# denyingmxd/CFPNet

Measured on AMD Instinct MI355X. Metric: depth maps/sec @ 480x640 bf16 (whole job; per_gpu = value / n_gpus); abs_rel vs CPU oracle, higher is better.
Workload: dtype bf16; 1 GPU; batch=8 480x640 RGB + 8x8-zone ToF, eval forward incl. the prob output [B,256,H/2,W/2] written in the storage dtype (bf16: 2 bytes/element); layers=hist2image combine1 image x2 (CFPNet), parallelism=single GPU

## Files before the change

cfpnet_amd/engine.py:

```python
from __future__ import annotations

import math
import os
from typing import Dict, List, Optional, Sequence, Tuple

import torch

from . import hip, ops, spec
from .geometry import FUSION_SCALES, FusionGeometry, gsa_keys, static_zone_key, zone_records as _zone_records
from .ops import Act

_BN_EPS = 1e-5


def _same_pad(size: int, k: int, s: int) -> Tuple[int, int]:
    total = max((math.ceil(size / s) - 1) * s + k - size, 0)
    return total // 2, total - total // 2


_STREAMS: Dict = {}
_CONCURRENT: Dict[str, list] = {}


def concurrent_streams(device, want: int = 4, pool: int = 16) -> list:
# ... 291 lines not shown
            bufs[key] = (torch.zeros if zero else torch.empty)(shape, dtype=dtype, device=self.device)
        assert tuple(bufs[key].shape) == tuple(shape), key
        return bufs[key]

    def _f32(self, plan, key: str, n: int) -> torch.Tensor:
        bufs = plan["bufs"]
        if key not in bufs:
            bufs[key] = torch.empty(max(n, 1), dtype=torch.float32, device=self.device)
        assert bufs[key].numel() >= n, key
        return bufs[key]

    def _cv(self, name, x: Act, out: Act, B, H, W, k, stride=1, pads=None, act=hip.ACT_NONE, residual=None):
        if pads is None:
            p = (k - 1) // 2
            pt = pl = p
            Ho, Wo = (H + 2 * p - k) // stride + 1, (W + 2 * p - k) // stride + 1
        else:
            (pt, pb), (pl, pr) = pads
            Ho, Wo = (H + pt + pb - k) // stride + 1, (W + pl + pr - k) // stride + 1
        ops.conv2d(x, self.P[name + ".w"], self.P[name + ".s"], self.P[name + ".t"], out, B, H, W, k, k, stride, pt, pl,
                   Ho, Wo, act, residual, self._ws(B * Ho * Wo, out.C, k * k * x.C))
        return Ho, Wo

    def _lin(self, wname, x: Act, out: Act, rows, act=hip.ACT_NONE, residual=None, st: Optional[str] = None, ln=None):
        ops.linear(x, self.P[wname], self.P[st + ".s"] if st else None, self.P[st + ".t"] if st else None, out, rows, act, residual,
                   None if ln is not None else self._ws(rows, out.C, x.C), ln)

    def _ws(self, M: int, Cout: int, K: int) -> Optional[torch.Tensor]:
        need = ops.conv2d_ws_bytes(M, Cout, K, self.cdt)
        if need == 0:
            return None
        if self.tickets:
            need += hip.CONV_TICKET_BYTES
        ws = self._lane_ws.get(self._lane)
        if ws is None or ws.numel() * 4 < need:
            if self._capturing:
                raise RuntimeError("split-K workspace must be sized by a warm-up forward before graph capture")
            if self.tickets:
                ws = ops.ticket_ws(need - hip.CONV_TICKET_BYTES, self.device)
            else:
                ws = torch.empty((need + 3) // 4, dtype=torch.float32, device=self.device)
            self._lane_ws[self._lane] = ws
        return ws

    def _dbg(self, name: str, a: Act):
        if self._dbg_round:
            for pat, dt in self._dbg_round.items():
                if name == pat or (pat.endswith("*") and name.startswith(pat[:-1])):
                    t = a.torch()
                    t.copy_(t.to(dt).to(t.dtype))

    def _encoder(self, plan, rgb: torch.Tensor, B, H, W, taps):
        e = "img_encoder"
        x8 = self._act(plan, "rgb8", B * H * W, 8)
        (ops.rgb_to_nhwc8_hilo if self.rgb_hilo else ops.rgb_to_nhwc8)(rgb, x8, B, H, W)
        pads = (_same_pad(H, 3, 2), _same_pad(W, 3, 2))
        h, w = math.ceil(H / 2), math.ceil(W / 2)
        x = self._act(plan, "stem", B * h * w, spec.ENC_STEM_OUT)
        self._cv("stem", x8, x, B, H, W, 3, 2, pads, hip.ACT_SILU if self.stem_act else hip.ACT_NONE)
        self._dbg("stem", x)
        tap_acts: List[Act] = []
        for bi, b in enumerate(spec.ENC_BLOCKS):
            q = f"{e}.{b.prefix}"
            ho, wo = math.ceil(h / b.stride), math.ceil(w / b.stride)
            pads = (_same_pad(h, 3, b.stride), _same_pad(w, 3, b.stride))
            if bi in spec.ENC_TAPS:
                out = plan["tap_dst"][spec.ENC_TAPS[bi]]
            else:
                out = self._act(plan, f"enc{bi}", B * ho * wo, b.cout)
            res = x if b.skip else None
            if b.kind == "cn":
                self._cv(q + ".conv", x, out, B, h, w, 3, b.stride, pads, hip.ACT_SILU, res)
            elif b.kind == "er":
                if (self.half and (q + ".pwl.wp") in self.P and ("1" if b.stride == 1 else "2") in self.er_fused and taps is None
                        and not self._dbg_round and ops.conv3x3_pw_fused_variant(x.C, b.mid, b.cout, b.stride, ops.DT[self.dtype]) >= 0):
                    ops.conv3x3_pw_fused(x, self.P[q + ".exp.w"], self.P[q + ".exp.s"], self.P[q + ".exp.t"], hip.ACT_SILU, self.P[q + ".pwl.wp"],
                                         self.P[q + ".pwl.s"], self.P[q + ".pwl.t"], out, B, h, w, b.stride, pads[0][0], pads[1][0], ho, wo,
                                         hip.ACT_NONE, res)
                else:
                    mid = self._act(plan, f"enc{bi}.mid", B * ho * wo, b.mid)
                    self._cv(q + ".exp", x, mid, B, h, w, 3, b.stride, pads, hip.ACT_SILU)
                    self._dbg(f"enc{bi}.mid", mid)
                    self._cv(q + ".pwl", mid, out, B, ho, wo, 1, 1, None, hip.ACT_NONE, res)
            else:
                mid2 = self._act(plan, f"enc{bi}.dw", B * ho * wo, b.mid)
                mbp = ops.mbconv_plan(B, h, w, x.C, b.mid) if (q + ".pw.wimg") in self.P else None
                if mbp is not None:
                    ns = mbp[0]
                    part = self._f32(plan, f"enc{bi}.sum", B * ns * b.mid)
                    ops.mbconv_expand_dw(x, self.P[q + ".pw.wimg"], self.P[q + ".pw.s"], self.P[q + ".pw.t"], self.P[q + ".dw.w"],
                                         self.P[q + ".dw.s"], self.P[q + ".dw.t"], mid2, part, B, h, w)
                elif ((self.se2 or self.se2_x3 == "1" or (self.se2_x3 == "auto" and not ops.PLAN_IN_FLIGHT)) and b.se_rd <= 64
                      and ops.dwconv3x3_se_parts(B, ho, wo, b.mid, b.stride, ops.DT[self.dtype]) > 0):
                    mid = self._act(plan, f"enc{bi}.mid", B * h * w, b.mid)
                    self._cv(q + ".pw", x, mid, B, h, w, 1, 1, None, hip.ACT_SILU)
                    K = ops.dwconv3x3_se_parts(B, ho, wo, b.mid, b.stride, ops.DT[self.dtype])
                    hpart = self._f32(plan, f"enc{bi}.hpart", B * K * b.se_rd)
                    ops.dwconv3x3_se(mid, self.P[q + ".dw.w"], self.P[q + ".dw.s"], self.P[q + ".dw.t"], mid2, self.P[q + ".se.wr"], hpart,
                                     B, h, w, b.stride, pads[0][0], pads[1][0], ho, wo, hip.ACT_SILU)
                    if self.x3:
                        wb = self._buf(plan, f"enc{bi}.wb", (B, b.cout, (b.mid + 31) // 32 * 64), torch.float16, zero=True)
                    else:
                        wb = self._buf(plan, f"enc{bi}.wb", (B, b.cout, b.mid), self.dtype)
                    ops.se_gate_fold2(hpart, K, 1.0 / (ho * wo), self.P[q + ".se.br"], self.P[q + ".se.we_t"], self.P[q + ".se.be"],
                                      self.P[q + ".pwl.w32"], wb, B, b.cout, b.mid, b.se_rd, x3=self.x3)
                    ops.conv2d(mid2, wb, self.P[q + ".pwl.s"], self.P[q + ".pwl.t"], out, B, ho, wo, 1, 1, 1, 0, 0, ho, wo, hip.ACT_NONE,
                               res, self._piw_ws(plan, bi, B, ho * wo, b.cout, b.mid), per_image_weights=True)
                    x, h, w = out, ho, wo
                    if bi in spec.ENC_TAPS:
                        tap_acts.append(out)
                        if taps is not None:
                            taps[f"enc{spec.ENC_TAPS[bi]}"] = self._nchw(out, B, h, w)
                    continue
                else:
                    mid = self._act(plan, f"enc{bi}.mid", B * h * w, b.mid)
                    self._cv(q + ".pw", x, mid, B, h, w, 1, 1, None, hip.ACT_SILU)
                    ns = ops.dwconv3x3_strips(B, ho, wo, b.mid, b.stride, ops.DT[self.dtype])
                    part = self._f32(plan, f"enc{bi}.sum", B * ns * b.mid)
                    self._dbg(f"enc{bi}.mid", mid)
                    ops.dwconv3x3_sum(mid, self.P[q + ".dw.w"], self.P[q + ".dw.s"], self.P[q + ".dw.t"], mid2, part, B, h, w, b.stride,
                                      pads[0][0], pads[1][0], ho, wo, hip.ACT_SILU)
                    self._dbg(f"enc{bi}.dw", mid2)
# ... 722 lines not shown
```

cfpnet_amd/hip.py:

```python
from __future__ import annotations

import ctypes as C
import os
from typing import Optional

_HERE = os.path.dirname(os.path.abspath(__file__))
LIB_PATH = os.environ.get("CFP_HIP_LIB") or os.path.join(_HERE, "libcfpnet_hip.so")

F32, BF16, F16 = 0, 1, 2
F32X3 = 3
ACT_NONE, ACT_RELU, ACT_LRELU, ACT_SILU, ACT_GELU, ACT_SIGMOID = range(6)
TOF_SAMPLE_UNIFORM, TOF_SAMPLE_ICDF = 0, 1
HEAD_WOUT_HILO, HEAD_RAM_HILO = 1, 2
UNC_STD, UNC_ENTROPY, UNC_PMAX = 0, 1, 2
SPARS_STD, SPARS_ENTROPY, SPARS_PMAX, SPARS_ORACLE_RMSE, SPARS_ORACLE_ABSREL = range(5)
RENDER_DEPTH, RENDER_GT, RENDER_ABS_ERR, RENDER_REL_ERR = range(4)
REGION_ALL, REGION_FOV_IN, REGION_FOV_OUT, REGION_ZONE_VALID, REGION_ZONE_INVALID = range(5)
CONV_PER_IMAGE, CONV_W2, CONV_IN_FLIGHT, CONV_X3, CONV_WS_TICKETS = 1, 2, 4, 8, 16
CONV_TICKET_BYTES = 4096

_p, _i, _f, _sz, _ll = C.c_void_p, C.c_int, C.c_float, C.c_size_t, C.c_longlong

SIGNATURES = {
    "cfp_version": (_i, []),
    "cfp_last_error": (C.c_char_p, []),
    "cfp_conv2d_nhwc": (_i, [_p, _i, _p, _p, _p, _p, _i, _p, _i] + [_i] * 14 + [_p, _sz, _p]),
    "cfp_conv2d_nhwc_ex": (_i, [_p, _i, _p, _p, _p, _p, _i, _p, _i] + [_i] * 14 + [_p, _p, _f, _i, _p, _sz, _p]),
    "cfp_conv2d_nhwc_moments": (_i, [_p, _i, _p, _p, _p, _i] + [_i] * 13 + [_p, _sz, _p, _sz, _p, _p, _p]),
    "cfp_conv2d_ws_bytes": (_sz, [_i, _i, _i, _i]),
    "cfp_pack_w_x3_elems": (_sz, [_ll, _i]),
    "cfp_pack_w_x3": (_i, [_p, _p, _ll, _i, _p]),
    "cfp_conv2d_plan": (_i, [_i] * 8 + [_p, _p]),
    "cfp_debug_set": (_i, [_i, _i]),
    "cfp_conv2d_variant": (_i, [_i, _i]),
    "cfp_dwconv3x3_nhwc": (_i, [_p, _i, _p, _p, _p, _p, _i] + [_i] * 11 + [_p]),
    "cfp_dwconv3x3_strips": (_i, [_i] * 6),
    "cfp_dwconv3x3_launch_slots": (_i, [_i] * 10),
    "cfp_dwconv3x3_sum_nhwc": (_i, [_p, _i, _p, _p, _p, _p, _i, _p] + [_i] * 11 + [_p]),
    "cfp_se_fold": (_i, [_p, _p, _p, _p, _p, _i, _i, _i, _i, _i, _p]),
    "cfp_se_gate_fold": (_i, [_p, _i, _f, _p, _p, _p, _p, _p, _p, _i, _i, _i, _i, _i, _p]),
    "cfp_dwconv3x3_se_parts": (_i, [_i, _i, _i, _i, _i, _i]),
    "cfp_dwconv3x3_se_nhwc": (_i, [_p, _i, _p, _p, _p, _p, _i, _p, _i, _p] + [_i] * 11 + [_p]),
    "cfp_se_gate_fold2": (_i, [_p, _i, _f, _p, _p, _p, _p, _p, _i, _i, _i, _i, _i, _p]),
    "cfp_dwconv_large_nhwc": (_i, [_p, _i, _p, _p, _p, _p, _i] + [_i] * 7 + [_p]),
    "cfp_dwconv_large_toeplitz_elems": (_sz, [_i, _i]),
    "cfp_dwconv_large_toeplitz": (_i, [_p, _p, _i, _i, _i, _i, _p]),
    "cfp_dwconv_large_mfma_nhwc": (_i, [_p, _i, _p, _p, _p, _p, _i] + [_i] * 7 + [_p]),
    "cfp_channel_sum": (_i, [_p, _i, _p, _i, _i, _i, _i, _i, _p]),
    "cfp_se_hidden": (_i, [_p, _i, _f, _p, _p, _p, _i, _i, _i, _p]),
    "cfp_se_scale": (_i, [_p, _i, _p, _p, _p, _i, _i, _i, _i, _i, _p]),
    "cfp_scale_channels": (_i, [_p, _i, _p, _i, _i, _i, _i, _p]),
    "cfp_layernorm": (_i, [_p, _i, _p, _p, _f, _p, _i, _p, _i, _i, _i, _i, _p]),
    "cfp_attn_kv_ws_floats": (_sz, [_i] * 7),
    "cfp_attn_kv_reduce": (_i, [_p, _i, _p, _i, _p, _p, _p] + [_i] * 10 + [_f, _i, _i, _i, _p]),
    "cfp_attn_apply": (_i, [_p, _i, _p, _p, _p, _i] + [_i] * 9 + [_f, _f, _i, _i, _i, _p]),
    "cfp_loftr_tail": (_i, [_p, _i, _p, _p, _p, _i, _p, _i, _p, _p, _p, _p, _p, _p, _p, _p, _f] + [_i] * 5 + [_f, _f, _i, _i, _i, _p]),
    "cfp_loftr_tail_x2i": (_i, [_p, _p, _p, _i, _i, _i, _i, _i] + [_p] * 8 + [_f] + [_i] * 5 + [_p, _i, _i, _f, _f, _i, _i, _i, _p]),
    "cfp_resize_bilinear": (_i, [_p, _i] + [_i] * 6 + [_p, _i] + [_i] * 6 + [_p] + [_i] * 7 + [_p]),
    "cfp_resize_bilinear_dev": (_i, [_p, _i, _i, _i, _p, _i, _i, _i, _p, _i, _p] + [_i] * 6 + [_i, _p]),
    "cfp_attn_kv_reduce_dev": (_i, [_p, _i, _p, _i, _p, _p, _p] + [_i] * 5 + [_p, _i, _i, _i, _i, _p]),
    "cfp_attn_kv_project_fits": (_i, [_i] * 8),
    "cfp_attn_kv_project_reduce": (_i, [_p, _i, _p, _p, _p, _p] + [_i] * 10 + [_f, _i, _i, _i, _p]),
    "cfp_attn_kv_project_reduce_dev": (_i, [_p, _i, _p, _p, _p, _p] + [_i] * 5 + [_p, _i, _i, _i, _i, _p]),
    "cfp_attn_apply_dev": (_i, [_p, _i, _p, _p, _p, _i] + [_i] * 5 + [_p, _f, _i, _i, _i, _p]),
    "cfp_add_rowtable": (_i, [_p, _i, _p, _p, _i] + [_i] * 8 + [_p]),
    "cfp_upsample_cat_conv3x3": (_i, [_p, _i, _i, _i, _i, _p, _i, _i, _p, _p, _p, _p, _i] + [_i] * 6 + [_p]),
# ... 45 lines not shown
    "cfp_bn_train_stats_partials": (_i, [_p, _i, C.c_longlong, C.c_longlong, _i, _p, _p, _f, _f] + [_p] * 7 + [_p]),
    "cfp_scale_shift_act": (_i, [_p, _i, _p, _p, _i, _p, _i, C.c_longlong, _i, _i, _p]),
    "cfp_scale_shift_act_res": (_i, [_p, _i, _p, _p, _i, _p, _i, _p, _i, C.c_longlong, _i, _i, _p]),
    "cfp_bn_train_bwd": (_i, [_p, _i, _p, _i, C.c_longlong, _i, _i, _p, _p, _p, _p, _i, _p, _p, _p, _i, _p, _sz, _p]),
    "cfp_colsum": (_i, [_p, _i, C.c_longlong, _i, _i, _p, _p, _sz, _p]),
    "cfp_act_bwd": (_i, [_p, _i, _p, _i, _i, _p, _i, C.c_longlong, _i, _i, _p]),
    "cfp_layernorm_bwd_ws_bytes": (_sz, [C.c_longlong, _i]),
    "cfp_layernorm_bwd": (_i, [_p, _i, _p, _i, _p, _f, _p, _i, _i, _p, _p, C.c_longlong, _i, _i, _p, _sz, _p]),
    "cfp_layernorm_bwd_deferred": (_i, [_p, _i, _p, _i, _p, _f, _p, _i, _i, _p, _p, C.c_longlong, _i, _i, _p, _sz, _p, _p]),
    "cfp_axpby": (_i, [_p, _i, _p, _i, _f, _f, _p, _i, C.c_longlong, _i, _i, _p]),
    "cfp_rowtable_grad": (_i, [_p, _i, _p, _i, _i, _i, _i, _i, _i, _i, _f, _i, _p]),
    "cfp_se_train_ws_floats": (_sz, [_i, _i, _i]),
    "cfp_se_train_fwd": (_i, [_p, _i, _f] + [_p] * 7 + [_i, _i, _i, _p]),
    "cfp_se_train_bwd": (_i, [_p] * 12 + [_f, _f, _i, _i, _i, _p]),
    "cfp_channel_dot": (_i, [_p, _i, _p, _i, _p, _i, _i, _i, _i, _p]),
    "cfp_bcast_fma": (_i, [_p, _i, _p, _p, _p, _i, _i, _i, _i, _i, _p]),
    "cfp_dwconv3x3_dgrad": (_i, [_p, _i, _p, _p, _i] + [_i] * 11 + [_p]),
    "cfp_dwconv3x3_wgrad_ws_bytes": (_sz, [_i]),
    "cfp_dwconv3x3_wgrad": (_i, [_p, _i, _p, _i, _p] + [_i] * 9 + [_f, _i, _p, _sz, _p]),
    "cfp_dwconv3x3_wgrad_deferred": (_i, [_p, _i, _p, _i, _p] + [_i] * 9 + [_f, _i, _p, _sz, _p, _p]),
    "cfp_index_rows": (_i, [_p, _i, _p, _p, _i, C.c_longlong, _i, _i, _i, _p]),
    "cfp_resize_bilinear_bwd": (_i, [_p, _i, _p, _i, _i, _i, _i, _i, _i, _i, _i, _i, _p]),
    "cfp_bin_centers": (_i, [_p, _f, _f, _p, _p, _i, _i, _p]),
    "cfp_bin_centers_bwd": (_i, [_p, _f, _f, _p, _i, _i, _p]),
    "cfp_softmax_expect_ws_bytes": (_sz, [_i, _i, _i]),
    "cfp_softmax_expect": (_i, [_p, _i, _p, _p, _p, _p, _i, _p, _i, _i, _i, _i, _p, _sz, _p]),
    "cfp_linattn_state_bytes": (_sz, [_i, _i, _i]),
    "cfp_linattn_ws_bytes": (_sz, [_i, _i, _i, _i, _i]),
    "cfp_linattn_fwd": (_i, [_p, _i, _p, _i, _p, _i, _p, _i, _p, _i, _i, _i, _i, _i, _f, _i, _p, _sz, _p]),
    "cfp_linattn_bwd": (_i, [_p, _i, _p, _i, _p, _i, _p, _i, _p, _p, _i, _p, _i, _p, _i, _i, _i, _i, _i, _i, _f, _i, _p, _sz, _p]),
    "cfp_linattn_fwd_dev": (_i, [_p, _i, _p, _i, _p, _i, _p, _i, _p, _i, _i, _i, _i, _i, _f, _i, _p, _sz, _p, _p]),
    "cfp_linattn_bwd_dev": (_i, [_p, _i, _p, _i, _p, _i, _p, _i, _p, _p, _i, _p, _i, _p, _i, _i, _i, _i, _i, _i, _f, _i, _p, _sz, _p, _p]),
    "cfp_zone_crop": (_i, [_p, _i, _p, _p, _i] + [_i] * 7 + [_i, _p]),
    "cfp_zone_crop_bwd": (_i, [_p, _i, _p, _p, _i] + [_i] * 7 + [_i, _p]),
    "cfp_zone_paste": (_i, [_p, _i, _p, _i, _p, _p, _i] + [_i] * 7 + [_i, _p]),
    "cfp_zone_paste_bwd": (_i, [_p, _i, _p, _p, _i] + [_i] * 7 + [_i, _p]),
    "cfp_zone_rect_rows": (_i, [_p, _i, _p, _p, _i] + [_i] * 6 + [_i, _p]),
    "cfp_dwconv_large_wgrad_ws_bytes": (_sz, [_i, _i, _i, _i, _i]),
    "cfp_dwconv_large_wgrad": (_i, [_p, _i, _p, _i, _p, _i, _i, _i, _i, _i, _f, _i, _p, _sz, _p]),
    "cfp_row_normalize": (_i, [_p, _p, _p, _i, _i, _p]),
    "cfp_add_rowtable_dev": (_i, [_p, _i, _p, _p, _i, _i, _i, _i, _i, _i, _i, _p, _i, _p]),
    "cfp_rowtable_grad_dev": (_i, [_p, _i, _p, _i, _i, _i, _i, _i, _i, _p, _f, _i, _p]),
    "cfp_nyu_augment": (_i, [_p, _p, _i, _i, _i, _p, _p, _p, _i, _i, C.POINTER(C.c_float), C.POINTER(C.c_float), _p, _p, _p]),
    "cfp_nyu_rotate": (_i, [_p, _p, _p, _p, _i, _i, _i, _p, _p]),
    "cfp_bin_regressor": (_i, [_p, _i, _f] + [_p] * 7 + [_f, _f, _i, _p, _p, _i, _i, _i, _i, _p]),
    "cfp_bin_softmax": (_i, [_p, _i, _p, _p, _p, _i, _i, _i, _i, _p]),
    "cfp_bin_softmax_stats": (_i, [_p, _i, _p, _p, _p, _p, _i, _i, _i, _i, _p]),
    "cfp_conv3x3_mean": (_i, [_p, _i, _p, _i, _p, _p, _p, _i, _i, _i, _i, _i, _i, _p]),
    "cfp_lkpm_tail": (_i, [_p, _i, _p, _i, _p, _i, _p, _p, _p, _p, _p, _p, _f, _i, _i, _i, _p]),
    "cfp_mbconv_plan": (_i, [_i, _i, _i, _i, _i, _p, _p]),
    "cfp_mbconv_expand_dw": (_i, [_p, _i, _p, _p, _p, _p, _p, _p, _p, _i, _p, _i, _i, _i, _i, _i, _i, _p]),
    "cfp_conv3x3_pw_fused_variant": (_i, [_i] * 5),
    "cfp_conv3x3_chunk_variant": (_i, [_i] * 4),
    "cfp_conv3x3_pw_fused": (_i, [_p, _i, _p, _p, _p, _i, _p, _p, _p, _i, _p, _i, _p, _i] + [_i] * 12 + [_p]),
    "cfp_hist_encoder": (_i, [_p, _p, _p, _p, _p, _p, _p, _p, _p, _i, _i, _i, _p]),
    "cfp_depth_head_fused": (_i, [_p, _i, _p, _p, _p, _p, _p, _p, _p, _p, _p, _i, _i, _i, _i, _i, _p]),
    "cfp_bin_head_fused": (_i, [_p, _i, _p, _p, _p, _p, _p, _i, _i, _i, _i, _p]),
    "cfp_depth_head_conv0_fused": (_i, [_p, _i, _p, _p, _p, _p, _p, _p, _p, _p, _p, _p, _p, _i, _i, _i, _i, _i, _p]),
    "cfp_depth_head_fused_stats": (_i, [_p, _i, _p, _p, _p, _p, _p, _p, _p, _p, _p, _p, _i, _i, _i, _i, _i, _p]),
    "cfp_bin_head_fused_stats": (_i, [_p, _i, _p, _p, _p, _p, _p, _p, _i, _i, _i, _i, _p]),
}

class WgradJob(C.Structure):
    _fields_ = [("slabs", C.c_void_p), ("dw", C.c_void_p), ("db", C.c_void_p), ("n", C.c_longlong), ("n_dw", C.c_longlong),
                ("nsplit", C.c_int), ("ew", C.c_int), ("beta", C.c_float), ("beta_b", C.c_float)]


_lib: Optional[C.CDLL] = None


def load() -> C.CDLL:
    global _lib
    if _lib is not None:
        return _lib
    if not os.path.exists(LIB_PATH):
        raise RuntimeError(
            f"{LIB_PATH} not found: build the HIP extension first "
            f"(`python -c 'import __graft_entry__ as g; g.build()'` or `make -C cfpnet_amd/csrc`). "
            "There is no CPU fallback for the product path.")
    import torch
    lib = C.CDLL(LIB_PATH)
    for name, (res, args) in SIGNATURES.items():
        fn = getattr(lib, name)
        fn.restype = res
        fn.argtypes = args
    _lib = lib
    return lib


def last_error() -> str:
    return load().cfp_last_error().decode()


def call(name: str, *args):
    rc = getattr(load(), name)(*args)
    if rc != 0:
        raise RuntimeError(f"{name} failed ({rc}): {last_error()}")


def ptr(t) -> int:
    return 0 if t is None else t.data_ptr()


def current_stream() -> int:
    import torch
    return torch.cuda.current_stream().cuda_stream
# ... 1 lines not shown
```

cfpnet_amd/ops.py:

```python
from __future__ import annotations

import os
from dataclasses import dataclass
from typing import Optional, Tuple

import torch

from . import hip

DT = {torch.float32: hip.F32, torch.bfloat16: hip.BF16, torch.float16: hip.F16}


@dataclass
class Act:
    buf: torch.Tensor
    c0: int
    C: int

    @property
    def rows(self) -> int:
        return self.buf.shape[0]

    @property
    def ld(self) -> int:
# ... 385 lines not shown
        hip.call("cfp_resize_bilinear_dev", src.ptr, src.ld, Hs, Ws, dst.ptr, dst.ld, Hd, Wd, _rec_ptr(rec), int(rec_side),
                 hip.ptr(zone_valid), zn, p1, p2, int(accumulate), B, src.C, src.dt, _s())
        return
    sy0, sx0, sh, sw = srect
    dy0, dx0, dh, dw = drect
    hip.call("cfp_resize_bilinear", src.ptr, src.ld, Hs, Ws, sy0, sx0, sh, sw, dst.ptr, dst.ld, Hd, Wd, dy0, dx0, dh, dw,
             hip.ptr(zone_valid), zn, p1, p2, int(accumulate), B, src.C, src.dt, _s())


def add_rowtable(x: Act, table, out: Act, rows, H, W, Wt, oy, ox):
    assert table.dtype == torch.float32 and table.shape[1] == x.C
    hip.call("cfp_add_rowtable", x.ptr, x.ld, table.data_ptr(), out.ptr, out.ld, rows, x.C, H, W, Wt, oy, ox, x.dt, _s())


def copy_rows(x: Act, out: Act, rows):
    hip.call("cfp_copy_rows", x.ptr, x.ld, out.ptr, out.ld, rows, x.C, x.dt, _s())


def upsample_cat_conv3x3(low: Act, Hs, Ws, skip: Act, w, scale, shift, out: Act, B, H, W, act, x3: bool = False):
    if x3:
        assert low.dt == skip.dt == out.dt == hip.F32 and w.dtype == torch.float16 and w.shape[-1] == 9 * (low.C + (skip.C + 31) // 32 * 32) * 2
        hip.call("cfp_upsample_cat_conv3x3", low.ptr, low.ld, Hs, Ws, low.C, skip.ptr, skip.ld, skip.C, w.data_ptr(),
                 hip.ptr(scale), hip.ptr(shift), out.ptr, out.ld, B, H, W, out.C, act, hip.F32X3, _s())
        return
    assert w.shape[-1] == 9 * (low.C + skip.C) and low.dt == skip.dt == out.dt
    hip.call("cfp_upsample_cat_conv3x3", low.ptr, low.ld, Hs, Ws, low.C, skip.ptr, skip.ld, skip.C, w.data_ptr(),
             hip.ptr(scale), hip.ptr(shift), out.ptr, out.ld, B, H, W, out.C, act, out.dt, _s())


def pack_w_x3_cat(w: torch.Tensor, cup: int) -> torch.Tensor:
    co, kh, kw, cin = w.shape
    assert kh == 3 and kw == 3 and cup % 32 == 0 and 0 < cup < cin
    csk = cin - cup
    pad = (csk + 31) // 32 * 32 - csk
    wp = torch.nn.functional.pad(w, (0, pad)) if pad else w
    return pack_w_x3(wp.reshape(co, 9 * (cup + csk + pad)).contiguous())


def copy_rows2(x0: Act, out0: Act, x1: Act, out1: Act, rows):
    assert x0.dt == x1.dt == out0.dt == out1.dt and out0.C == x0.C and out1.C == x1.C
    hip.call("cfp_copy_rows2", x0.ptr, x0.ld, out0.ptr, out0.ld, x0.C, x1.ptr, x1.ld, out1.ptr, out1.ld, x1.C, rows, x0.dt, _s())


def rgb_to_nhwc8(rgb: torch.Tensor, out: Act, B, H, W):
    assert rgb.dtype == torch.float32 and rgb.is_contiguous() and out.C == 8 and out.ld == 8
    hip.call("cfp_rgb_to_nhwc8", rgb.data_ptr(), out.ptr, B, H, W, out.dt, _s())


def rgb_to_nhwc8_hilo(rgb: torch.Tensor, out: Act, B, H, W):
    assert rgb.dtype == torch.float32 and rgb.is_contiguous() and out.C == 8 and out.ld == 8
    hip.call("cfp_rgb_to_nhwc8_hilo", rgb.data_ptr(), out.ptr, B, H, W, out.dt, _s())


def scalar_to_rows8(x: torch.Tensor, out: Act, rows):
    assert x.dtype == torch.float32 and x.is_contiguous() and out.C == 8 and out.ld == 8
    hip.call("cfp_scalar_to_rows8", x.data_ptr(), out.ptr, rows, out.dt, _s())


def bin_regressor(partial, nsplit, inv_hw, w1x1, w0, b0, w1, b1, w2, b2, min_val, max_val, norm, edges, centers, B, C,
                  hidden, nbins):
    hip.call("cfp_bin_regressor", partial.data_ptr(), nsplit, float(inv_hw), w1x1.data_ptr(), w0.data_ptr(), b0.data_ptr(),
             w1.data_ptr(), b1.data_ptr(), w2.data_ptr(), b2.data_ptr(), float(min_val), float(max_val), norm,
             edges.data_ptr(), centers.data_ptr(), B, C, hidden, nbins, _s())


def _check_stats(stats, B, HW):
    assert stats.dtype == torch.float32 and stats.is_contiguous() and stats.numel() == B * 3 * HW, "stats: float32 [B, 3, HW]"


def bin_softmax(logits: Act, centers, prob, pred, B, HW, nbins, stats=None):
    if stats is None:
        hip.call("cfp_bin_softmax", logits.ptr, logits.ld, centers.data_ptr(), hip.ptr(prob), pred.data_ptr(), B, HW, nbins,
                 logits.dt, _s())
        return
    _check_stats(stats, B, HW)
    hip.call("cfp_bin_softmax_stats", logits.ptr, logits.ld, centers.data_ptr(), hip.ptr(prob), pred.data_ptr(), stats.data_ptr(), B, HW,
             nbins, logits.dt, _s())


def bin_head_fused(x: Act, w, bias, centers, prob, pred, B, HW, stats=None):
    x3 = x.buf.dtype == torch.float32 and w.dtype == torch.float16
    assert not x3 or (tuple(w.shape) == (256, (x.C + 31) // 32 * 64) and (prob is None or prob.dtype == torch.float32))
    if stats is None:
        hip.call("cfp_bin_head_fused", x.ptr, x.ld, w.data_ptr(), bias.data_ptr(), centers.data_ptr(), hip.ptr(prob),
                 pred.data_ptr(), B, HW, x.C, hip.F32X3 if x3 else x.dt, _s())
        return
    _check_stats(stats, B, HW)
    hip.call("cfp_bin_head_fused_stats", x.ptr, x.ld, w.data_ptr(), bias.data_ptr(), centers.data_ptr(), hip.ptr(prob),
             pred.data_ptr(), stats.data_ptr(), B, HW, x.C, hip.F32X3 if x3 else x.dt, _s())


def permute_wout(w: torch.Tensor, dtype, hilo: bool = True, diffuse: bool = False) -> torch.Tensor:
    w = w.detach().float().reshape(w.shape[0], -1)
    assert w.shape == (256, 128)
    src = pw_k_order(128)
    wp = w[:, src]
    hi = (round_taps(w.reshape(256, 1, 128), dtype).reshape(256, 128)[:, src] if diffuse else wp).to(dtype)
    planes = [hi]
    if hilo:
        planes.append((wp - hi.float()).to(dtype))
    return torch.stack(planes).contiguous()


def pw_k_order(K: int) -> torch.Tensor:
    pos = torch.arange((K + 31) // 32 * 32)
    kb, q, e = pos // 32, (pos % 32) // 8, pos % 8
# ... 103 lines not shown
```

include/cfpnet_hip.h:

```cpp
#ifndef CFPNET_HIP_H
#define CFPNET_HIP_H

#include <stddef.h>
#include <stdint.h>

#ifdef __cplusplus
extern "C" {
#endif

typedef void* cfp_stream_t;

enum { CFP_OK = 0, CFP_EINVAL = -1, CFP_ESHAPE = -2, CFP_EHIP = -3 };
enum { CFP_F32 = 0, CFP_BF16 = 1, CFP_F16 = 2 };
enum { CFP_F32X3 = 3 };
enum { CFP_TOF_SAMPLE_UNIFORM = 0, CFP_TOF_SAMPLE_ICDF = 1 };
enum { CFP_ACT_NONE = 0, CFP_ACT_RELU = 1, CFP_ACT_LRELU = 2, CFP_ACT_SILU = 3, CFP_ACT_GELU = 4, CFP_ACT_SIGMOID = 5 };

int cfp_version(void);
const char* cfp_last_error(void);

int cfp_conv2d_nhwc(const void* in, int in_ld, const void* w, const float* scale, const float* shift,
                    const void* residual, int res_ld, void* out, int out_ld,
                    int B, int H, int W, int Cin, int Cout, int KH, int KW, int stride,
                    int pad_t, int pad_l, int Ho, int Wo, int act, int dtype,
// ... 14 lines not shown
size_t cfp_conv2d_ws_bytes(int M, int Cout, int K, int dtype);

int cfp_conv2d_plan(int M, int Cout, int K, int KH, int stride, int dtype, int rows_per_batch, int B, int* variant,
                    int* splits);

int cfp_conv3x3_chunk_variant(int M, int Cin, int Cout, int in_flight);

int cfp_conv2d_variant(int M, int Cout);

int cfp_debug_set(int key, int value);

int cfp_dwconv3x3_nhwc(const void* in, int in_ld, const void* w, const float* scale, const float* shift,
                       void* out, int out_ld, int B, int H, int W, int C, int stride, int pad_t, int pad_l,
                       int Ho, int Wo, int act, int dtype, cfp_stream_t stream);

int cfp_dwconv3x3_strips(int B, int Ho, int Wo, int C, int stride, int dtype);
int cfp_dwconv3x3_launch_slots(int B, int H, int W, int Ho, int Wo, int C, int stride, int in_ld, int out_ld, int dtype);
int cfp_dwconv3x3_sum_nhwc(const void* in, int in_ld, const void* w, const float* scale, const float* shift,
                           void* out, int out_ld, float* partial, int B, int H, int W, int C, int stride,
                           int pad_t, int pad_l, int Ho, int Wo, int act, int dtype, cfp_stream_t stream);

int cfp_dwconv_large_nhwc(const void* in, int in_ld, const float* w, const float* scale, const float* shift,
                          void* out, int out_ld, int B, int H, int W, int C, int k, int act, int dtype,
                          cfp_stream_t stream);

size_t cfp_dwconv_large_toeplitz_elems(int C, int k);
int cfp_dwconv_large_toeplitz(const float* w, void* out, int C, int k, int flip, int dtype, cfp_stream_t stream);
int cfp_dwconv_large_mfma_nhwc(const void* in, int in_ld, const void* toeplitz, const float* scale, const float* shift,
                               void* out, int out_ld, int B, int H, int W, int C, int k, int act, int dtype,
                               cfp_stream_t stream);

int cfp_channel_sum(const void* in, int in_ld, float* partial, int B, int HW, int C, int nsplit, int dtype,
                    cfp_stream_t stream);

int cfp_se_hidden(const float* partial, int nsplit, float inv_hw, const float* w_reduce, const float* b_reduce,
                  float* hidden, int B, int C, int R, cfp_stream_t stream);

int cfp_se_scale(void* x, int ld, const float* hidden, const float* w_expand_t, const float* b_expand,
                 int B, int HW, int C, int R, int dtype, cfp_stream_t stream);

int cfp_se_fold(const void* w_proj, void* w_out, const float* hidden, const float* w_expand_t, const float* b_expand,
                int B, int Cout, int C, int R, int dtype, cfp_stream_t stream);

int cfp_mbconv_plan(int B, int H, int W, int Cin, int mid, int* tiles_per_image, int* KP);
int cfp_mbconv_expand_dw(const void* x, int x_ld, const void* wpw, const float* s1, const float* t1, const void* wdw,
                         const float* s2, const float* t2, void* out, int out_ld, float* partial, int B, int H, int W, int Cin,
                         int mid, int dtype, cfp_stream_t stream);

int cfp_conv3x3_pw_fused_variant(int Cin, int Cmid, int Cout, int stride, int dtype);
int cfp_conv3x3_pw_fused(const void* in, int in_ld, const void* w1, const float* scale1, const float* shift1, int act1,
                         const void* w2_pad, const float* scale2, const float* shift2, int act2, const void* residual, int res_ld,
                         void* out, int out_ld, int B, int H, int W, int Cin, int Cmid, int Cout, int stride, int pad_t, int pad_l,
                         int Ho, int Wo, int dtype, cfp_stream_t stream);

int cfp_se_gate_fold(const float* partial, int nsplit, float inv_hw, const float* w_reduce, const float* b_reduce,
                     const float* w_expand_t, const float* b_expand, const void* w_proj, void* w_out,
                     int B, int Cout, int C, int R, int dtype, cfp_stream_t stream);

int cfp_dwconv3x3_se_parts(int B, int Ho, int Wo, int C, int stride, int dtype);
int cfp_dwconv3x3_se_nhwc(const void* in, int in_ld, const void* w, const float* scale, const float* shift, void* out, int out_ld,
                          const float* w_reduce, int R, float* hpart, int B, int H, int W, int C, int stride, int pad_t, int pad_l,
                          int Ho, int Wo, int act, int dtype, cfp_stream_t stream);

int cfp_se_gate_fold2(const float* hpart, int K, float inv_hw, const float* b_reduce, const float* w_expand_t, const float* b_expand,
                      const float* w_proj, void* w_out, int B, int Cout, int C, int R, int dtype, cfp_stream_t stream);

int cfp_scale_channels(void* x, int ld, const float* gate, int B, int HW, int C, int dtype, cfp_stream_t stream);

int cfp_layernorm(const void* in, int in_ld, const float* gamma, const float* beta, float eps,
                  const void* residual, int res_ld, void* out, int out_ld, int rows, int C, int dtype,
                  cfp_stream_t stream);

size_t cfp_attn_kv_ws_floats(int NB, int Hk, int Wk, int th, int tw, int heads, int d);
int cfp_attn_kv_reduce(const void* k, int k_ld, const void* v, int v_ld, float* kv, float* ksum, float* ws,
                       int NB, int Hk, int Wk, int th, int tw, int cy0, int cy1, int cx0, int cx1,
                       int count_pad, float v_length, int heads, int d, int dtype, cfp_stream_t stream);

int cfp_attn_kv_reduce_dev(const void* k, int k_ld, const void* v, int v_ld, float* kv, float* ksum, float* ws,
                           int NB, int Hk, int Wk, int th, int tw, const int* rec, int count_pad, int heads, int d, int dtype,
                           cfp_stream_t stream);

int cfp_attn_kv_project_fits(int NB, int Hk, int Wk, int th, int tw, int heads, int d, int dtype);
int cfp_attn_kv_project_reduce(const void* x, int x_ld, const void* w_kv, float* kv, float* ksum, float* ws,
                               int NB, int Hk, int Wk, int th, int tw, int cy0, int cy1, int cx0, int cx1,
                               int count_pad, float v_length, int heads, int d, int dtype, cfp_stream_t stream);
int cfp_attn_kv_project_reduce_dev(const void* x, int x_ld, const void* w_kv, float* kv, float* ksum, float* ws,
                                   int NB, int Hk, int Wk, int th, int tw, const int* rec, int count_pad, int heads, int d, int dtype,
                                   cfp_stream_t stream);

int cfp_attn_apply(const void* q, int q_ld, const float* kv, const float* ksum, void* out, int out_ld,
                   int NB, int Hq, int Wq, int qth, int qtw, int ey0, int ey1, int ex0, int ex1,
                   float v_length, float eps, int heads, int d, int dtype, cfp_stream_t stream);

int cfp_attn_apply_dev(const void* q, int q_ld, const float* kv, const float* ksum, void* out, int out_ld,
                       int NB, int Hq, int Wq, int qth, int qtw, const int* rec, float eps, int heads, int d, int dtype,
                       cfp_stream_t stream);

int cfp_loftr_tail(const void* q, int q_ld, const float* kv, const float* ksum, const void* x, int x_ld,
                   void* out, int out_ld, const void* w_q, const void* w_merge, const void* w_mlp0, const void* w_mlp2,
                   const float* ln1_g, const float* ln1_b, const float* ln2_g, const float* ln2_b, float ln_eps,
                   int NB, int Hq, int Wq, int qth, int qtw, float v_length, float eps, int heads, int D,
                   int dtype, cfp_stream_t stream);

int cfp_loftr_tail_x2i(const float* kv, const float* ksum, void* tok, int tok_ld, int H, int W, int sy, int sx,
                       const void* w_q, const void* w_merge, const void* w_mlp0, const void* w_mlp2,
                       const float* ln1_g, const float* ln1_b, const float* ln2_g, const float* ln2_b, float ln_eps,
// ... 286 lines not shown
```

Measured before the change: 4093 maps/s.

## Fuse RGB hi/lo packing, stem conv and first encoder conv into one kernel

Adds a HIP kernel that reads fp32 RGB directly, splits it into hi/lo half-precision pairs in LDS, runs the stride-2 stem 3x3 conv with MFMA into an LDS tile with halo, then runs the first 3x3 conv block from LDS and writes only its 16-channel output. This removes the rgb8 and 40-channel stem activation round trips through global memory and two kernel launches. In exchange it recomputes the stem on halo pixels per tile and uses a large LDS footprint, which may limit occupancy. It is enabled by default for half dtypes with hilo RGB, and an environment variable can turn it off.

```diff
diff --git a/cfpnet_amd/csrc/stem_fused.hip b/cfpnet_amd/csrc/stem_fused.hip
--- /dev/null
+++ b/cfpnet_amd/csrc/stem_fused.hip
@@ -0,0 +1,270 @@
+#include "halo_core.h"
+
+namespace {
+
+constexpr int kC0 = 40, kK0 = 72;
+constexpr int kC1 = 16, kK1 = 9 * kC0;
+constexpr int kPP = 96;
+constexpr int kRC = 37;
+constexpr int kW0Bytes = kC0 * kK0 * 2, kW1Bytes = kC1 * kK1 * 2;
+constexpr int kNK = 2 * kC0 + 2 * kC1;
+
+struct StemP {
+  const float* rgb;
+  const void* w0;
+  const float *s0, *t0;
+  const void* w1;
+  const float *s1, *t1;
+  void* out;
+  int out_ld, H, W, Hs, Ws, tiles_x, tiles_y, act0, act1;
+  int probe;
+};
+
+template <int TH> struct StemTile {
+  static constexpr int SR = TH + 2, SPIX = SR * 18;
+  static constexpr int RR = 2 * SR + 1, RPIX = RR * kRC;
+  static constexpr int S_BYTES = SPIX * kPP, RGB_BYTES = RPIX * 16;
+  static constexpr int K_OFF = S_BYTES + (RGB_BYTES + kW0Bytes > kW1Bytes ? RGB_BYTES + kW0Bytes : kW1Bytes);
+  static constexpr int LDS = K_OFF + kNK * 4;
+};
+
+template <typename H, int TH>
+__global__ __launch_bounds__(256) void stem_fused_kernel(StemP p) {
+  using T = StemTile<TH>;
+  constexpr int SPIX = T::SPIX, RPIX = T::RPIX;
+  constexpr int NR = (RPIX + 255) / 256;
+  constexpr int RW = TH / 4;
+  static_assert(kW1Bytes / 16 <= 3 * 256 && kW0Bytes / 16 <= 2 * 256, "weight pieces per thread");
+  __shared__ __attribute__((aligned(16))) unsigned char smem[T::LDS];
+  unsigned char* sS = smem;
+  unsigned char* sR = smem + T::S_BYTES;
+  unsigned char* sW0 = sR + T::RGB_BYTES;
+  unsigned char* sW1 = sR;
+  float* sK = reinterpret_cast<float*>(smem + T::K_OFF);
+
+  const int tid = threadIdx.x;
+  const int lane = tid & 63;
+  const int wave = __builtin_amdgcn_readfirstlane(tid >> 6);
+  const int fr = lane & 15, fq = lane >> 4;
+
+  int bid = xcd_remap(blockIdx.x, gridDim.x);
+  const int x0 = (bid % p.tiles_x) * 16; bid /= p.tiles_x;
+  const int y0 = (bid % p.tiles_y) * TH;
+  const int b = bid / p.tiles_y;
+  const int HW = p.H * p.W;
+
+  u32x4 w1r[3], w0r[2];
+#pragma unroll
+  for (int n = 0; n < 3; ++n) {
+    const int i = tid + n * 256;
+    w1r[n] = i < kW1Bytes / 16 ? reinterpret_cast<const u32x4*>(p.w1)[i] : u32x4{0u, 0u, 0u, 0u};
+  }
+#pragma unroll
+  for (int n = 0; n < 2; ++n) {
+    const int i = tid + n * 256;
+    w0r[n] = i < kW0Bytes / 16 ? reinterpret_cast<const u32x4*>(p.w0)[i] : u32x4{0u, 0u, 0u, 0u};
+  }
+
+  float kv = 0.f;
+  {
+    const float* src = nullptr;
+    int k = tid;
+    if (k < kC0) { src = p.s0; kv = 1.f; }
+    else if ((k -= kC0) < kC0) src = p.t0;
+    else if ((k -= kC0) < kC1) { src = p.s1; kv = 1.f; }
+    else if ((k -= kC1) < kC1) src = p.t1;
+    if (src) kv = src[k];
+  }
+
+  {
+    const float* __restrict__ img = p.rgb + (long long)b * 3 * HW;
+    const int iy0 = 2 * (y0 - 1), ix0 = 2 * (x0 - 1);
+    float f[NR][3];
+#pragma unroll
+    for (int n = 0; n < NR; ++n) {
+      const int i = tid + n * 256;
+      const int r = i / kRC, q = i - r * kRC;
+      const int y = iy0 + r, x = ix0 + q;
+      const bool ok = i < RPIX && (unsigned)y < (unsigned)p.H && (unsigned)x < (unsigned)p.W;
+      const int o = ok ? y * p.W + x : 0;
+#pragma unroll
+      for (int c = 0; c < 3; ++c) f[n][c] = ok ? img[c * HW + o] : 0.f;
+    }
+#pragma unroll
+    for (int n = 0; n < NR; ++n) {
+      const int i = tid + n * 256;
+      if (i >= RPIX) continue;
+      float v[8];
+#pragma unroll
+      for (int c = 0; c < 3; ++c) {
+        const float x = f[n][c];
+        const float hi = to_f32<H>(from_f32<H>(x));
+        v[c] = hi;
+        v[3 + c] = x - hi;
+      }
+      v[6] = 0.f; v[7] = 0.f;
+      Vec<H>::store(reinterpret_cast<H*>(sR + i * 16), v);
+    }
+#pragma unroll
+    for (int n = 0; n < 2; ++n) {
+      const int i = tid + n * 256;
+      if (i < kW0Bytes / 16) *reinterpret_cast<u32x4*>(sW0 + i * 16) = w0r[n];
+    }
+    if (tid < kNK) sK[tid] = kv;
+  }
+  __syncthreads();
+  if (p.probe == 1) {
+    if (*reinterpret_cast<const volatile unsigned*>(sR + tid * 4) == 0x7fc12345u) reinterpret_cast<H*>(p.out)[0] = from_f32<H>(0.f);
+    return;
+  }
+
+  {
+    const s16x8 zero = {0, 0, 0, 0, 0, 0, 0, 0};
+    s16x8 wf[3][3];
+    int toff[3];
+#pragma unroll
+    for (int st = 0; st < 3; ++st) {
+      const int c = 4 * st + fq;
+      const bool live = c < 9;
+      const int dy = c / 3, dx = c - dy * 3;
+      toff[st] = live ? (dy * kRC + dx) * 16 : -1;
+#pragma unroll
+      for (int j = 0; j < 3; ++j) {
+        const int n = 16 * j + fr;
+        wf[st][j] = (live && n < kC0) ? *reinterpret_cast<const s16x8*>(sW0 + n * (kK0 * 2) + c * 16) : zero;
+      }
+    }
+    f32x4 sc[3], sh[3];
+#pragma unroll
+    for (int j = 0; j < 3; ++j) {
+      const int n = 16 * j + 4 * fq;
+      const bool ok = n < kC0;
+      sc[j] = ok ? *reinterpret_cast<const f32x4*>(sK + n) : f32x4{1.f, 1.f, 1.f, 1.f};
+      sh[j] = ok ? *reinterpret_cast<const f32x4*>(sK + kC0 + n) : f32x4{0.f, 0.f, 0.f, 0.f};
+    }
+    constexpr int NG = (SPIX + 15) / 16;
+    for (int g = wave; g < NG; g += 4) {
+      const int pix = 16 * g + fr;
+      const bool pv = pix < SPIX;
+      const int pc = pv ? pix : 0;
+      const int hy = pc / 18, hx = pc - hy * 18;
+      const unsigned char* base = sR + ((2 * hy) * kRC + 2 * hx) * 16;
+      f32x4 acc[3];
+#pragma unroll
+      for (int j = 0; j < 3; ++j) acc[j] = f32x4{0.f, 0.f, 0.f, 0.f};
+#pragma unroll
+      for (int st = 0; st < 3; ++st) {
+        const s16x8 xf = *reinterpret_cast<const s16x8*>(toff[st] >= 0 ? base + toff[st] : sR);
+#pragma unroll
+        for (int j = 0; j < 3; ++j) acc[j] = mfma16<H>(wf[st][j], xf, acc[j]);
+      }
+      const int sy = y0 - 1 + hy, sx = x0 - 1 + hx;
+      const bool inmap = (unsigned)sy < (unsigned)p.Hs && (unsigned)sx < (unsigned)p.Ws;
+      with_act(p.act0, [&](auto A) {
+#pragma unroll
+        for (int j = 0; j < 3; ++j) {
+          const int n = 16 * j + 4 * fq;
+          float yv[4];
+#pragma unroll
+          for (int r = 0; r < 4; ++r) yv[r] = act_c16<decltype(A)::value>(acc[j][r] * sc[j][r] + sh[j][r]);
+          uint2 pk;
+          pk.x = pack2<H>(yv[0], yv[1]);
+          pk.y = pack2<H>(yv[2], yv[3]);
+          if (!inmap) pk = uint2{0u, 0u};
+          if (pv && n < kC0) *reinterpret_cast<uint2*>(sS + pix * kPP + n * 2) = pk;
+        }
+      });
+    }
+  }
+  __syncthreads();
+#pragma unroll
+  for (int n = 0; n < 3; ++n) {
+    const int i = tid + n * 256;
+    if (i < kW1Bytes / 16) *reinterpret_cast<u32x4*>(sW1 + i * 16) = w1r[n];
+  }
+  __syncthreads();
+  if (p.probe == 2) {
+    if (*reinterpret_cast<const volatile unsigned*>(sS + tid * 4) == 0x7fc12345u) reinterpret_cast<H*>(p.out)[0] = from_f32<H>(0.f);
+    return;
+  }
+
+  f32x4 acc[RW];
+#pragma unroll
+  for (int g = 0; g < RW; ++g) acc[g] = f32x4{0.f, 0.f, 0.f, 0.f};
+  {
+    const s16x8 zero = {0, 0, 0, 0, 0, 0, 0, 0};
+    constexpr int CPT = kC0 / 8;
+    const unsigned char* xrow = sS + ((wave * RW) * 18 + fr) * kPP;
+    const unsigned char* wrow = sW1 + fr * (kK1 * 2);
+#pragma unroll
+    for (int st = 0; st < (9 * CPT + 3) / 4; ++st) {
+      const int c = 4 * st + fq;
+      const bool live = c < 9 * CPT;
+      const int tap = c / CPT, cc = c - tap * CPT;
+      const int dy = tap / 3, dx = tap - dy * 3;
+      const int xo = (dy * 18 + dx) * kPP + cc * 16;
+      const s16x8 wf = live ? *reinterpret_cast<const s16x8*>(wrow + c * 16) : zero;
+#pragma unroll
+      for (int g = 0; g < RW; ++g) {
+        const s16x8 xf = *reinterpret_cast<const s16x8*>(live ? xrow + g * 18 * kPP + xo : sS);
+        acc[g] = mfma16<H>(wf, xf, acc[g]);
+      }
+    }
+  }
+
+  H* __restrict__ out = reinterpret_cast<H*>(p.out) + (long long)b * p.Hs * p.Ws * p.out_ld;
+  const int n = 4 * fq, x = x0 + fr;
+  const f32x4 sc = *reinterpret_cast<const f32x4*>(sK + 2 * kC0 + n);
+  const f32x4 sh = *reinterpret_cast<const f32x4*>(sK + 2 * kC0 + kC1 + n);
+  with_act(p.act1, [&](auto A) {
+#pragma unroll
+    for (int g = 0; g < RW; ++g) {
+      const int y = y0 + wave * RW + g;
+      float yv[4];
+#pragma unroll
+      for (int r = 0; r < 4; ++r) yv[r] = act_c16<decltype(A)::value>(acc[g][r] * sc[r] + sh[r]);
+      uint2 pk;
+      pk.x = pack2<H>(yv[0], yv[1]);
+      pk.y = pack2<H>(yv[2], yv[3]);
+      if (y < p.Hs && x < p.Ws) *reinterpret_cast<uint2*>(out + ((long long)y * p.Ws + x) * p.out_ld + n) = pk;
+    }
+  });
+}
+
+template <typename H, int TH> void launch_stem(StemP p, int B, hipStream_t s) {
+  p.tiles_x = cdiv(p.Ws, 16); p.tiles_y = cdiv(p.Hs, TH);
+  hipLaunchKernelGGL((stem_fused_kernel<H, TH>), dim3((unsigned)(B * p.tiles_x * p.tiles_y)), dim3(256), 0, s, p);
+}
+
+}
+
+extern "C" int cfp_stem_fused_fits(int H, int W, int dtype) {
+  return is16(dtype) && H >= 2 && W >= 2 && H % 2 == 0 && W % 2 == 0 && 3ll * H * W < (1ll << 31) ? 1 : 0;
+}
+
+extern "C" int cfp_stem_fused(const float* rgb, const void* w_stem, const float* scale_stem, const float* shift_stem, int act_stem, const void* w1,
+                              const float* scale1, const float* shift1, int act1, void* out, int out_ld, int B, int H, int W, int Cstem, int Cout,
+                              int flags, int dtype, cfp_stream_t stream) {
+  static_assert(kPP == 96, "pitch");
+  CFP_REQUIRE(rgb && w_stem && w1 && out, CFP_EINVAL, "cfp_stem_fused: null pointer");
+  CFP_REQUIRE(is16(dtype), CFP_ESHAPE, "cfp_stem_fused: bf16 / f16 storage only");
+  CFP_REQUIRE(act_stem >= CFP_ACT_NONE && act_stem <= CFP_ACT_SIGMOID && act1 >= CFP_ACT_NONE && act1 <= CFP_ACT_SIGMOID, CFP_EINVAL,
+              "cfp_stem_fused: bad activation");
+  CFP_REQUIRE(B > 0 && cfp_stem_fused_fits(H, W, dtype), CFP_ESHAPE, "cfp_stem_fused: shape not taken (cfp_stem_fused_fits: even H, W >= 2)");
+  CFP_REQUIRE(Cstem == kC0 && Cout == kC1, CFP_ESHAPE, "cfp_stem_fused: the stem has 40 output channels and conv0.2.0 has 16");
+  CFP_REQUIRE(out_ld % 4 == 0 && out_ld >= Cout, CFP_ESHAPE, "cfp_stem_fused: out_ld must be a multiple of 4 and cover the channels");
+  CFP_REQUIRE((long long)B * (H / 2) * (W / 2) < (1ll << 31) && (long long)B * cdiv(H / 2, 8) * cdiv(W / 2, 16) < (1ll << 31), CFP_ESHAPE,
+              "cfp_stem_fused: problem too large");
+  CFP_REQUIRE((reinterpret_cast<uintptr_t>(rgb) & 3) == 0 && aligned16(w_stem) && aligned16(w1) && aligned16(scale_stem) && aligned16(shift_stem) &&
+                  aligned16(scale1) && aligned16(shift1) && (reinterpret_cast<uintptr_t>(out) & 7) == 0,
+              CFP_EINVAL, "cfp_stem_fused: weights and per-channel vectors must be 16-byte aligned, out 8-byte aligned");
+  CFP_REQUIRE(halo16_pitch(kC0, 1, false) == kPP, CFP_EHIP, "cfp_stem_fused: the tile pitch left the halo kernel's rule");
+  StemP p{};
+  p.rgb = rgb; p.w0 = w_stem; p.s0 = scale_stem; p.t0 = shift_stem; p.w1 = w1; p.s1 = scale1; p.t1 = shift1; p.out = out;
+  p.out_ld = out_ld; p.H = H; p.W = W; p.Hs = H / 2; p.Ws = W / 2; p.act0 = act_stem; p.act1 = act1; p.probe = flags & 3;
+  hipStream_t s = reinterpret_cast<hipStream_t>(stream);
+  const bool big = (flags & CFP_STEM_TILE16) != 0;
+  if (dtype == CFP_F16) { if (big) launch_stem<f16_t, 16>(p, B, s); else launch_stem<f16_t, 8>(p, B, s); }
+  else { if (big) launch_stem<bf16_t, 16>(p, B, s); else launch_stem<bf16_t, 8>(p, B, s); }
+  return cfp_check_launch("cfp_stem_fused");
+}
diff --git a/cfpnet_amd/engine.py b/cfpnet_amd/engine.py
--- a/cfpnet_amd/engine.py
+++ b/cfpnet_amd/engine.py
@@ -367,13 +367,19 @@
 
     def _encoder(self, plan, rgb: torch.Tensor, B, H, W, taps):
         e = "img_encoder"
-        x8 = self._act(plan, "rgb8", B * H * W, 8)
-        (ops.rgb_to_nhwc8_hilo if self.rgb_hilo else ops.rgb_to_nhwc8)(rgb, x8, B, H, W)
-        pads = (_same_pad(H, 3, 2), _same_pad(W, 3, 2))
         h, w = math.ceil(H / 2), math.ceil(W / 2)
-        x = self._act(plan, "stem", B * h * w, spec.ENC_STEM_OUT)
-        self._cv("stem", x8, x, B, H, W, 3, 2, pads, hip.ACT_SILU if self.stem_act else hip.ACT_NONE)
-        self._dbg("stem", x)
+        b0 = spec.ENC_BLOCKS[0]
+        stem_fused = (self.half and self.rgb_hilo and taps is None and not self._dbg_round and os.environ.get("CFP_STEM_FUSED", "1") != "0"
+                      and b0.kind == "cn" and b0.stride == 1 and not b0.skip and 0 not in spec.ENC_TAPS and ops.stem_fused_fits(H, W, self.dtype))
+        if stem_fused:
+            x = None
+        else:
+            x8 = self._act(plan, "rgb8", B * H * W, 8)
+            (ops.rgb_to_nhwc8_hilo if self.rgb_hilo else ops.rgb_to_nhwc8)(rgb, x8, B, H, W)
+            pads = (_same_pad(H, 3, 2), _same_pad(W, 3, 2))
+            x = self._act(plan, "stem", B * h * w, spec.ENC_STEM_OUT)
+            self._cv("stem", x8, x, B, H, W, 3, 2, pads, hip.ACT_SILU if self.stem_act else hip.ACT_NONE)
+            self._dbg("stem", x)
         tap_acts: List[Act] = []
         for bi, b in enumerate(spec.ENC_BLOCKS):
             q = f"{e}.{b.prefix}"
@@ -383,6 +389,11 @@
                 out = plan["tap_dst"][spec.ENC_TAPS[bi]]
             else:
                 out = self._act(plan, f"enc{bi}", B * ho * wo, b.cout)
+            if bi == 0 and stem_fused:
+                ops.stem_fused(rgb, self.P["stem.w"], self.P["stem.s"], self.P["stem.t"], hip.ACT_SILU if self.stem_act else hip.ACT_NONE,
+                               self.P[q + ".conv.w"], self.P[q + ".conv.s"], self.P[q + ".conv.t"], hip.ACT_SILU, out, B, H, W)
+                x = out
+                continue
             res = x if b.skip else None
             if b.kind == "cn":
                 self._cv(q + ".conv", x, out, B, h, w, 3, b.stride, pads, hip.ACT_SILU, res)
diff --git a/cfpnet_amd/hip.py b/cfpnet_amd/hip.py
--- a/cfpnet_amd/hip.py
+++ b/cfpnet_amd/hip.py
@@ -12,6 +12,7 @@
 ACT_NONE, ACT_RELU, ACT_LRELU, ACT_SILU, ACT_GELU, ACT_SIGMOID = range(6)
 TOF_SAMPLE_UNIFORM, TOF_SAMPLE_ICDF = 0, 1
 HEAD_WOUT_HILO, HEAD_RAM_HILO = 1, 2
+STEM_TILE16 = 16
 UNC_STD, UNC_ENTROPY, UNC_PMAX = 0, 1, 2
 SPARS_STD, SPARS_ENTROPY, SPARS_PMAX, SPARS_ORACLE_RMSE, SPARS_ORACLE_ABSREL = range(5)
 RENDER_DEPTH, RENDER_GT, RENDER_ABS_ERR, RENDER_REL_ERR = range(4)
@@ -163,6 +164,8 @@
     "cfp_mbconv_expand_dw": (_i, [_p, _i, _p, _p, _p, _p, _p, _p, _p, _i, _p, _i, _i, _i, _i, _i, _i, _p]),
     "cfp_conv3x3_pw_fused_variant": (_i, [_i] * 5),
     "cfp_conv3x3_chunk_variant": (_i, [_i] * 4),
+    "cfp_stem_fused_fits": (_i, [_i] * 3),
+    "cfp_stem_fused": (_i, [_p, _p, _p, _p, _i, _p, _p, _p, _i, _p] + [_i] * 8 + [_p]),
     "cfp_conv3x3_pw_fused": (_i, [_p, _i, _p, _p, _p, _i, _p, _p, _p, _i, _p, _i, _p, _i] + [_i] * 12 + [_p]),
     "cfp_hist_encoder": (_i, [_p, _p, _p, _p, _p, _p, _p, _p, _p, _i, _i, _i, _p]),
     "cfp_depth_head_fused": (_i, [_p, _i, _p, _p, _p, _p, _p, _p, _p, _p, _p, _i, _i, _i, _i, _i, _p]),
diff --git a/cfpnet_amd/ops.py b/cfpnet_amd/ops.py
--- a/cfpnet_amd/ops.py
+++ b/cfpnet_amd/ops.py
@@ -461,6 +461,19 @@
     hip.call("cfp_rgb_to_nhwc8_hilo", rgb.data_ptr(), out.ptr, B, H, W, out.dt, _s())
 
 
+def stem_fused_fits(H: int, W: int, dtype) -> bool:
+    return dtype in DT and bool(hip.load().cfp_stem_fused_fits(H, W, DT[dtype]))
+
+
+def stem_fused(rgb: torch.Tensor, w_stem: torch.Tensor, s_stem, t_stem, act_stem, w1: torch.Tensor, s1, t1, act1, out: Act, B, H, W,
+               tile16: bool = False, probe: int = 0):
+    assert rgb.dtype == torch.float32 and rgb.is_contiguous() and rgb.numel() == B * 3 * H * W and out.rows >= B * (H // 2) * (W // 2)
+    assert w_stem.dtype == out.buf.dtype and w_stem.is_contiguous() and w_stem.shape[1] == 72
+    assert w1.dtype == out.buf.dtype and w1.is_contiguous() and tuple(w1.shape) == (out.C, 9 * w_stem.shape[0])
+    hip.call("cfp_stem_fused", rgb.data_ptr(), w_stem.data_ptr(), hip.ptr(s_stem), hip.ptr(t_stem), act_stem, w1.data_ptr(), hip.ptr(s1),
+             hip.ptr(t1), act1, out.ptr, out.ld, B, H, W, w_stem.shape[0], out.C, (hip.STEM_TILE16 if tile16 else 0) | probe, out.dt, _s())
+
+
 def scalar_to_rows8(x: torch.Tensor, out: Act, rows):
     assert x.dtype == torch.float32 and x.is_contiguous() and out.C == 8 and out.ld == 8
     hip.call("cfp_scalar_to_rows8", x.data_ptr(), out.ptr, rows, out.dt, _s())
diff --git a/include/cfpnet_hip.h b/include/cfpnet_hip.h
--- a/include/cfpnet_hip.h
+++ b/include/cfpnet_hip.h
@@ -90,6 +90,12 @@
                          const void* w2_pad, const float* scale2, const float* shift2, int act2, const void* residual, int res_ld,
                          void* out, int out_ld, int B, int H, int W, int Cin, int Cmid, int Cout, int stride, int pad_t, int pad_l,
                          int Ho, int Wo, int dtype, cfp_stream_t stream);
+
+enum { CFP_STEM_TILE16 = 16 };
+int cfp_stem_fused_fits(int H, int W, int dtype);
+int cfp_stem_fused(const float* rgb, const void* w_stem, const float* scale_stem, const float* shift_stem, int act_stem, const void* w1,
+                   const float* scale1, const float* shift1, int act1, void* out, int out_ld, int B, int H, int W, int Cstem, int Cout,
+                   int flags, int dtype, cfp_stream_t stream);
 
 int cfp_se_gate_fold(const float* partial, int nsplit, float inv_hw, const float* w_reduce, const float* b_reduce,
                      const float* w_expand_t, const float* b_expand, const void* w_proj, void* w_out,
```

New measurement: 4132 maps/s, median of 6. No clear change (+1.0%).
